# johnnyjana730/MVIN

Hardware: AMD Instinct MI355X
Metric: (user,item) pairs scored/sec @ dim=64 hop=2 fan-out=32; % HBM roofline (higher is better)
Workload: dtype f32

## Files before the change

### mvin_amd/csrc/mvin_keyaddr_flash.hip

```cpp
#include <cstdlib>
#include <type_traits>

#include "mvin_kernels.h"

namespace mvin {

typedef float f32x4 __attribute__((ext_vector_type(4)));

constexpr int kFlashChunk = 64;
constexpr int kFlashWaves = 4;

__global__ void ka_flash_slots_kernel(const int32_t* __restrict__ seg_ptr, const int32_t* __restrict__ nseg_dev, int nseg_bound,
                                      int32_t* __restrict__ slot_seg) {
    const int nseg = nseg_dev ? min(*nseg_dev, nseg_bound) : nseg_bound;
    for (int s = blockIdx.x * blockDim.x + threadIdx.x; s < nseg; s += gridDim.x * blockDim.x) {
        const int p0 = seg_ptr[s], p1 = seg_ptr[s + 1];
        const int first = p0 / kFlashChunk + s;
        const int nch = (p1 - p0 + kFlashChunk - 1) / kFlashChunk;
        for (int c = 0; c < nch; ++c) slot_seg[first + c] = s;
    }
}

#define KAF_FENCE() __builtin_amdgcn_sched_barrier(0)

__device__ long long g_kaf_trace[64 * 16];

template <int NMT, bool HAS_SET, bool TRACE = false>
__global__ __launch_bounds__(kFlashWaves * 64, 2) void key_addr_flash_kernel(KaFlashArgs a, KaRecLayout RL) {
    constexpr int D = 64;
    __shared__ f32x4 sUo0[kFlashWaves][4][64];
    const int lane = threadIdx.x & 63, l16 = lane & 15, q16 = lane >> 4;
    f32x4 (*myUo0)[64] = sUo0[threadIdx.x >> 6];
    const int P = a.P, NmP = RL.NmP;
    const unsigned emax = (unsigned)(a.n_entity - 1);
    const float* __restrict__ E = a.E;
    const size_t tw_stride = (size_t)a.n_entity * D;

    struct Rows {
        float4 v[NMT][4];
    };
    auto issue_u = [&](int mt, const int (&hr)[NMT], Rows& R) {
        const f32x4* src = reinterpret_cast<const f32x4*>(a.ER + (size_t)(unsigned)max(hr[mt], 0) * D) + q16;
#pragma unroll
        for (int nt = 0; nt < 4; ++nt) {
            const f32x4 v = __builtin_nontemporal_load(src + 4 * nt);
            R.v[mt][nt] = make_float4(v[0], v[1], v[2], v[3]);
        }
    };
    auto issue_t = [&](int mt, const float* __restrict__ tab, const int4 (&ids)[NMT], Rows& R) {
        const int id[4] = {ids[mt].x, ids[mt].y, ids[mt].z, ids[mt].w};
#pragma unroll
        for (int i = 0; i < 4; ++i)
            R.v[mt][i] = reinterpret_cast<const float4*>(tab + (size_t)(unsigned)max(id[i], 0) * D)[l16];
    };
    auto reads_tile = [&](bool two, int mt, const Rows& R, const f32x4 (&p0)[NMT], const f32x4 (&p1)[NMT], f32x4 (&u0)[4], f32x4 (&u1)[4]) {
        if (two) {
#pragma unroll
            for (int i = 0; i < 4; ++i) {
                const float t[4] = {R.v[mt][i].x, R.v[mt][i].y, R.v[mt][i].z, R.v[mt][i].w};
#pragma unroll
                for (int nt = 0; nt < 4; ++nt) u0[nt] = __builtin_amdgcn_mfma_f32_16x16x4f32(t[nt], p0[mt][i], u0[nt], 0, 0, 0);
#pragma unroll
                for (int nt = 0; nt < 4; ++nt) u1[nt] = __builtin_amdgcn_mfma_f32_16x16x4f32(t[nt], p1[mt][i], u1[nt], 0, 0, 0);
            }
        } else {
#pragma unroll
            for (int i = 0; i < 4; ++i) {
                const float t[4] = {R.v[mt][i].x, R.v[mt][i].y, R.v[mt][i].z, R.v[mt][i].w};
#pragma unroll
                for (int nt = 0; nt < 4; ++nt) u0[nt] = __builtin_amdgcn_mfma_f32_16x16x4f32(t[nt], p0[mt][i], u0[nt], 0, 0, 0);
            }
        }
    };
    auto softmax = [&](f32x4 (&lg)[NMT], const int4 (&ids)[NMT]) {
        float mx = -INFINITY;
#pragma unroll
        for (int mt = 0; mt < NMT; ++mt) {
            const int id[4] = {ids[mt].x, ids[mt].y, ids[mt].z, ids[mt].w};
#pragma unroll
            for (int i = 0; i < 4; ++i) mx = fmaxf(mx, id[i] >= 0 ? lg[mt][i] : -INFINITY);
        }
        mx = xor32_max(xor16_max(mx));
        float z = 0.f;
#pragma unroll
        for (int mt = 0; mt < NMT; ++mt) {
            const int id[4] = {ids[mt].x, ids[mt].y, ids[mt].z, ids[mt].w};
#pragma unroll
            for (int i = 0; i < 4; ++i) {
                const float x = lean_exp(fminf(lg[mt][i] - mx, 0.f));
                const float e = id[i] >= 0 ? x : 0.f;
                lg[mt][i] = e;
                z += e;
            }
        }
        z = xor32_sum(xor16_sum(z));
        const float inv = 1.f / z;
#pragma unroll
        for (int mt = 0; mt < NMT; ++mt) {
#pragma unroll
            for (int i = 0; i < 4; ++i) lg[mt][i] *= inv;
        }
    };

    int iter = 0;
    auto stamp = [&](int slot) {
        if constexpr (TRACE) {
            if (blockIdx.x == 0 && threadIdx.x == 0 && iter >= 2 && iter < 66) g_kaf_trace[(iter - 2) * 16 + slot] = __builtin_readcyclecounter();
        }
    };
    for (;; ++iter) {
        stamp(0);
        int k = 0;
        if (lane == 0) k = atomicAdd(a.counter, 1) + 1;
        k = __builtin_amdgcn_readfirstlane(k);
        if (k >= a.nslots) break;
        const int s = __builtin_amdgcn_readfirstlane(a.slot_seg[k]);
        if (s < 0) continue;
        const int u = __builtin_amdgcn_readfirstlane(a.seg_user[s]);
        const int p0 = __builtin_amdgcn_readfirstlane(a.seg_ptr[s]), p1 = __builtin_amdgcn_readfirstlane(a.seg_ptr[s + 1]);
        const int cbeg = p0 + (k - (p0 / kFlashChunk + s)) * kFlashChunk;
        const int cend = min(p1, cbeg + kFlashChunk);
        const int32_t* __restrict__ rec = a.records + (size_t)u * RL.len;
        stamp(1);
        auto load_hr = [&](int hop, int (&hr)[NMT]) {
#pragma unroll
            for (int mt = 0; mt < NMT; ++mt) hr[mt] = rec[RL.o_hr + hop * NmP + 16 * mt + l16];
        };
        auto load_tid = [&](int hop, int4 (&tid)[NMT]) {
#pragma unroll
            for (int mt = 0; mt < NMT; ++mt) tid[mt] = *reinterpret_cast<const int4*>(rec + RL.o_tail + hop * NmP + 16 * mt + 4 * q16);
        };
        auto load_orig = [&](int t0, int (&orig)[2], bool (&valid)[2]) {
#pragma unroll
            for (int rt = 0; rt < 2; ++rt) {
                const int p = t0 + 16 * rt + l16;
                valid[rt] = p < cend;
                orig[rt] = a.pair_index[min(p, cend - 1)];
            }
        };
        auto load_item = [&](const int (&orig)[2], unsigned (&item)[2]) {
#pragma unroll
            for (int rt = 0; rt < 2; ++rt)
                item[rt] = min(a.items64 ? reinterpret_cast<const unsigned*>(a.items64)[2 * (int64_t)orig[rt]] : (unsigned)a.items32[orig[rt]], emax);
        };
        auto load_be = [&](const unsigned (&item)[2], float4 (&bE)[2][4]) {
#pragma unroll
            for (int rt = 0; rt < 2; ++rt) {
#pragma unroll
                for (int nt = 0; nt < 4; ++nt) bE[rt][nt] = reinterpret_cast<const float4*>(E + (size_t)item[rt] * D)[4 * nt + q16];
            }
        };

        int orig[2], origN[2];
        bool valid[2], validN[2];
        unsigned item[2];
        float4 bE[2][4];
        int hrC[NMT], hrN[NMT];
        int4 tidC[NMT];
        Rows R;
        load_orig(cbeg, orig, valid);
        load_hr(0, hrC);
        load_tid(0, tidC);
        load_orig(cbeg + 32, origN, validN);
        f32x4 uo0[4];
#pragma unroll
        for (int r = 0; r < 4; ++r) {
            const float4 b = a.bmlp ? reinterpret_cast<const float4*>(a.bmlp)[4 * q16 + r] : make_float4(0.f, 0.f, 0.f, 0.f);
            uo0[0][r] = b.x, uo0[1][r] = b.y, uo0[2][r] = b.z, uo0[3][r] = b.w;
        }
        if constexpr (HAS_SET) {
            int4 hid[NMT];
            f32x4 ph[NMT];
#pragma unroll
            for (int mt = 0; mt < NMT; ++mt) hid[mt] = *reinterpret_cast<const int4*>(rec + RL.o_head + 16 * mt + 4 * q16);
#pragma unroll
            for (int mt = 0; mt < NMT; ++mt) issue_t(mt, a.TW, hid, R);
            KAF_FENCE();
            stamp(11);
#pragma unroll
            for (int mt = 0; mt < NMT; ++mt) {
                const int id[4] = {hid[mt].x, hid[mt].y, hid[mt].z, hid[mt].w};
#pragma unroll
                for (int i = 0; i < 4; ++i) ph[mt][i] = a.hs[max(id[i], 0)];
            }
            load_item(orig, item);
            KAF_FENCE();
            stamp(12);
            softmax(ph, hid);
            KAF_FENCE();
            stamp(13);
            f32x4 unused[4];
#pragma unroll
            for (int mt = 0; mt < NMT; ++mt) {
                reads_tile(false, mt, R, ph, ph, uo0, unused);
                KAF_FENCE();
                issue_u(mt, hrC, R);
                KAF_FENCE();
            }
            stamp(14);
        } else {
            load_item(orig, item);
#pragma unroll
            for (int mt = 0; mt < NMT; ++mt) issue_u(mt, hrC, R);
        }
        load_be(item, bE);
#pragma unroll
        for (int nt = 0; nt < 4; ++nt) myUo0[nt][lane] = uo0[nt];
        KAF_FENCE();
        stamp(2);

        const int ntile = (cend - cbeg + 31) >> 5;
        int t0 = cbeg;
        auto run_tile = [&](const bool two, const bool more) {
            f32x4 uo[2][4];
#pragma unroll
            for (int rt = 0; rt < 2; ++rt) {
#pragma unroll
                for (int nt = 0; nt < 4; ++nt) uo[rt][nt] = myUo0[nt][lane];
            }
            unsigned itemN[2];
            if (more) load_item(origN, itemN);
            for (int hop = 0; hop < P; ++hop) {
                const bool last_hop = hop + 1 == P;
                const bool next_stage = !last_hop || more;
                const int hopN = last_hop ? 0 : hop + 1;
                const float* __restrict__ tw = a.TW + (size_t)(hop + (HAS_SET ? 1 : 0)) * tw_stride;
                if (next_stage) load_hr(hopN, hrN);
                KAF_FENCE();
                if (t0 == cbeg && hop < 3) stamp(3 + 4 * hop);
                f32x4 lg[2][NMT];
#pragma unroll
                for (int mt = 0; mt < NMT; ++mt) {
                    lg[0][mt] = f32x4{0.f, 0.f, 0.f, 0.f};
                    lg[1][mt] = f32x4{0.f, 0.f, 0.f, 0.f};
                    if (two) {
#pragma unroll
                        for (int nt = 0; nt < 4; ++nt) {
                            const float av[4] = {R.v[mt][nt].x, R.v[mt][nt].y, R.v[mt][nt].z, R.v[mt][nt].w};
                            const float e0[4] = {bE[0][nt].x, bE[0][nt].y, bE[0][nt].z, bE[0][nt].w};
                            const float e1[4] = {bE[1][nt].x, bE[1][nt].y, bE[1][nt].z, bE[1][nt].w};
#pragma unroll
                            for (int i = 0; i < 4; ++i) {
                                lg[0][mt] = __builtin_amdgcn_mfma_f32_16x16x4f32(av[i], e0[i], lg[0][mt], 0, 0, 0);
                                lg[1][mt] = __builtin_amdgcn_mfma_f32_16x16x4f32(av[i], e1[i], lg[1][mt], 0, 0, 0);
                            }
                        }
                    } else {
#pragma unroll
                        for (int nt = 0; nt < 4; ++nt) {
                            const float av[4] = {R.v[mt][nt].x, R.v[mt][nt].y, R.v[mt][nt].z, R.v[mt][nt].w};
                            const float e0[4] = {bE[0][nt].x, bE[0][nt].y, bE[0][nt].z, bE[0][nt].w};
#pragma unroll
                            for (int i = 0; i < 4; ++i) lg[0][mt] = __builtin_amdgcn_mfma_f32_16x16x4f32(av[i], e0[i], lg[0][mt], 0, 0, 0);
                        }
                    }
                    KAF_FENCE();
                    issue_t(mt, tw, tidC, R);
                    KAF_FENCE();
                }
                if (last_hop && more) load_be(itemN, bE);
                KAF_FENCE();
                if (t0 == cbeg && hop < 3) stamp(4 + 4 * hop);
                softmax(lg[0], tidC);
                if (two) softmax(lg[1], tidC);
                KAF_FENCE();
                if (t0 == cbeg && hop < 3) stamp(5 + 4 * hop);
#pragma unroll
                for (int mt = 0; mt < NMT; ++mt) {
                    reads_tile(two, mt, R, lg[0], lg[1], uo[0], uo[1]);
                    KAF_FENCE();
                    if (next_stage) issue_u(mt, hrN, R);
                    KAF_FENCE();
                }
                if (next_stage) load_tid(hopN, tidC);
                if (t0 == cbeg && hop < 3) stamp(6 + 4 * hop);
            }
#pragma unroll
            for (int rt = 0; rt < 2; ++rt) {
                if (valid[rt] && (rt == 0 || two)) {
#pragma unroll
                    for (int r = 0; r < 4; ++r)
                        *reinterpret_cast<float4*>(a.user_o + (size_t)orig[rt] * D + 16 * q16 + 4 * r) =
                            make_float4(uo[rt][0][r], uo[rt][1][r], uo[rt][2][r], uo[rt][3][r]);
                }
            }
        };
        for (int tile = 0; tile < ntile; ++tile, t0 += 32) {
            const bool more = tile + 1 < ntile;
            run_tile(cend - t0 > 16, more);
#pragma unroll
            for (int rt = 0; rt < 2; ++rt) orig[rt] = origN[rt], valid[rt] = validN[rt];
        }
        stamp(15);
    }
}

hipError_t kaf_read_trace(long long* host_dst, size_t n) {
    const size_t have = sizeof(g_kaf_trace) / sizeof(long long);
    return hipMemcpyFromSymbol(host_dst, HIP_SYMBOL(g_kaf_trace), (n < have ? n : have) * sizeof(long long));
}
#undef KAF_FENCE

bool key_addr_flash_supported(int D, int P, int Nm, int nR, int n_entity) {
    if (D != 64 || P < 1 || P > 8 || Nm < 1 || Nm > 64) return false;
    const KaRecLayout RL = ka_rec_layout(P, Nm, nR);
    if (RL.len == 0) return false;
    return (long long)nR * n_entity < (1ll << 31);
}

size_t key_addr_flash_ws_elems(int64_t B, int nseg_bound) { return (size_t)(B / kFlashChunk + nseg_bound + 1) + 1; }

template <int NMT>
static hipError_t launch_flash_n(const KaFlashArgs& a, const KaRecLayout& RL, bool has_set, hipStream_t st) {
    auto k = has_set ? key_addr_flash_kernel<NMT, true> : key_addr_flash_kernel<NMT, false>;
    if constexpr (NMT == 4) {
        static const bool trace = getenv("MVIN_KAF_TRACE") != nullptr;
        if (trace && has_set) k = key_addr_flash_kernel<4, true, true>;
    }
    static thread_local int per_cu[2] = {0, 0};
    int& pc = per_cu[has_set ? 1 : 0];
    if (pc == 0) {
        int v = 0;
        if (hipOccupancyMaxActiveBlocksPerMultiprocessor(&v, reinterpret_cast<const void*>(k), kFlashWaves * 64, 0) != hipSuccess || v < 1) v = 2;
        pc = v > 8 ? 8 : v;
    }
    const int64_t want = ((int64_t)a.nslots + kFlashWaves - 1) / kFlashWaves;
    const int grid = (int)(want < 256 * (int64_t)pc ? want : 256 * (int64_t)pc);
    k<<<grid, kFlashWaves * 64, 0, st>>>(a, RL);
    return hipGetLastError();
}

hipError_t launch_key_addr_flash(const KaFlashArgs& a_, int nseg_bound, bool has_set, int32_t* sched_ws, hipStream_t st) {
    KaFlashArgs a = a_;
    const KaRecLayout RL = ka_rec_layout(a.P, a.Nm, a.nR);
    if (RL.len == 0 || !sched_ws) return hipErrorInvalidValue;
    a.nslots = (int)(a.B / kFlashChunk + nseg_bound + 1);
    a.slot_seg = sched_ws;
    a.counter = sched_ws + a.nslots;
    hipError_t e = hipMemsetAsync(sched_ws, 0xFF, ((size_t)a.nslots + 1) * sizeof(int32_t), st);
    if (e != hipSuccess) return e;
    {
        const int blocks = nseg_bound < 256 * 64 ? (nseg_bound + 255) / 256 : 64;
        ka_flash_slots_kernel<<<blocks > 0 ? blocks : 1, 256, 0, st>>>(a.seg_ptr, a.nseg_dev, nseg_bound, sched_ws);
        e = hipGetLastError();
        if (e != hipSuccess) return e;
    }
    switch (RL.NmP / 16) {
        case 1: return launch_flash_n<1>(a, RL, has_set, st);
        case 2: return launch_flash_n<2>(a, RL, has_set, st);
        case 3: return launch_flash_n<3>(a, RL, has_set, st);
        case 4: return launch_flash_n<4>(a, RL, has_set, st);
        default: return hipErrorInvalidValue;
    }
}

}
```

Measured before the change: 514.2 million.

## Prefetch next work item's records into LDS with static slot schedule

Replaces the atomic work counter with a static strided slot assignment per wave, and software-pipelines the next item's scheduling metadata, user record (head/tail/hr ids) and pair indices into double-buffered LDS via global_load_lds while the current item computes. Per-item index loads then come from LDS instead of global memory, hiding the dependent-load latency at item start. It also drops the nontemporal hint on relation-row loads and replaces the null-bias branch with a zero device buffer. The cost is LDS use that may lower occupancy, and static scheduling loses the dynamic load balancing the atomic counter gave.

Measured after the change: 534.4 million, median of 6. +3.9%, better.

```diff
diff --git a/mvin_amd/csrc/mvin_keyaddr_flash.hip b/mvin_amd/csrc/mvin_keyaddr_flash.hip
--- a/mvin_amd/csrc/mvin_keyaddr_flash.hip
+++ b/mvin_amd/csrc/mvin_keyaddr_flash.hip
@@ -23,9 +23,12 @@
 
 #define KAF_FENCE() __builtin_amdgcn_sched_barrier(0)
 
+__device__ float g_kaf_no_bias[64];
 __device__ long long g_kaf_trace[64 * 16];
 
-template <int NMT, bool HAS_SET, bool TRACE = false>
+extern __shared__ __attribute__((aligned(16))) int32_t sKafRec[];
+
+template <int NMT, bool HAS_SET, bool PF, bool TRACE = false>
 __global__ __launch_bounds__(kFlashWaves * 64, 2) void key_addr_flash_kernel(KaFlashArgs a, KaRecLayout RL) {
     constexpr int D = 64;
     __shared__ f32x4 sUo0[kFlashWaves][4][64];
@@ -34,6 +37,7 @@
     const int P = a.P, NmP = RL.NmP;
     const unsigned emax = (unsigned)(a.n_entity - 1);
     const float* __restrict__ E = a.E;
+    const float* __restrict__ bias = a.bmlp;
     const size_t tw_stride = (size_t)a.n_entity * D;
 
     struct Rows {
@@ -43,7 +47,7 @@
         const f32x4* src = reinterpret_cast<const f32x4*>(a.ER + (size_t)(unsigned)max(hr[mt], 0) * D) + q16;
 #pragma unroll
         for (int nt = 0; nt < 4; ++nt) {
-            const f32x4 v = __builtin_nontemporal_load(src + 4 * nt);
+            const f32x4 v = src[4 * nt];
             R.v[mt][nt] = make_float4(v[0], v[1], v[2], v[3]);
         }
     };
@@ -108,27 +112,147 @@
             if (blockIdx.x == 0 && threadIdx.x == 0 && iter >= 2 && iter < 66) g_kaf_trace[(iter - 2) * 16 + slot] = __builtin_readcyclecounter();
         }
     };
+    auto load_item_raw = [&](const int (&orig)[2], unsigned (&item)[2]) {
+#pragma unroll
+        for (int rt = 0; rt < 2; ++rt)
+            item[rt] = a.items64 ? reinterpret_cast<const unsigned*>(a.items64)[2 * (int64_t)orig[rt]] : (unsigned)a.items32[orig[rt]];
+    };
+    auto load_item = [&](const int (&orig)[2], unsigned (&item)[2]) {
+        load_item_raw(orig, item);
+#pragma unroll
+        for (int rt = 0; rt < 2; ++rt) item[rt] = min(item[rt], emax);
+    };
+
+    const int wave = __builtin_amdgcn_readfirstlane((int)(threadIdx.x >> 6));
+    const int stride = (int)gridDim.x * kFlashWaves;
+    const int recW = (1 + 2 * P) * NmP, ldsT = NmP, ldsHr = NmP + P * NmP;
+    const unsigned lds0 = (unsigned)(size_t)(__attribute__((address_space(3))) char*)sKafRec + (unsigned)(wave * 2 * recW * 4);
+    const int lorig = kFlashWaves * 2 * recW + wave * 32;
+    const unsigned ldsOrig = (unsigned)(size_t)(__attribute__((address_space(3))) char*)sKafRec + (unsigned)(lorig * 4);
+    auto la_slots_issue = [&](long long base) -> int {
+        const long long kc = base + (long long)stride * (lane + 1);
+        return kc < a.nslots ? a.slot_seg[kc] : -1;
+    };
+    auto la_slots_take = [&](long long base, int sv, int& kN, int& sN) -> bool {
+        for (;;) {
+            const unsigned long long live = __ballot(sv >= 0);
+            if (live) {
+                const int j = __ffsll(live) - 1;
+                kN = __builtin_amdgcn_readfirstlane((int)(base + (long long)stride * (j + 1)));
+                sN = __builtin_amdgcn_readlane(sv, j);
+                return true;
+            }
+            base += 64ll * stride;
+            if (base + stride >= a.nslots) return false;
+            sv = la_slots_issue(base);
+        }
+    };
+    auto la_seg_issue = [&](int s) -> int {
+        const int32_t* src = lane == 0 ? a.seg_user + s : a.seg_ptr + s + (lane - 1);
+        return lane < 3 ? *src : 0;
+    };
+    auto la_seg_take = [&](int v, int k, int s, int& u, int& cbeg, int& cend) {
+        u = __builtin_amdgcn_readlane(v, 0);
+        const int p0 = __builtin_amdgcn_readlane(v, 1), p1 = __builtin_amdgcn_readlane(v, 2);
+        cbeg = p0 + (k - (p0 / kFlashChunk + s)) * kFlashChunk;
+        cend = min(p1, cbeg + kFlashChunk);
+    };
+    auto la_rec_issue = [&](int u, int cbeg, int cend, int par) {
+        const char* src = reinterpret_cast<const char*>(a.records + (size_t)u * RL.len);
+        const unsigned dst = lds0 + (unsigned)(par * recW * 4);
+        for (int j0 = 0; j0 < recW; j0 += 64) {
+            const int i = j0 + lane;
+            if (i < recW) {
+                const int voff = 4 * (i < NmP ? RL.o_head + i : RL.o_tail + (i - NmP));
+                unsigned keep;
+                asm volatile("s_nop 4\n\ts_mov_b32 %0, m0\n\ts_mov_b32 m0, %3\n\ts_nop 0\n\tglobal_load_lds_dword %1, %2\n\ts_mov_b32 m0, %0"
+                             : "=&s"(keep)
+                             : "v"(voff), "s"(src), "s"(dst + 4u * (unsigned)j0)
+                             : "memory");
+            }
+        }
+        if (lane < 32) {
+            const int voff = 4 * min(lane, cend - 1 - cbeg);
+            unsigned keep;
+            asm volatile("s_nop 4\n\ts_mov_b32 %0, m0\n\ts_mov_b32 m0, %3\n\ts_nop 0\n\tglobal_load_lds_dword %1, %2\n\ts_mov_b32 m0, %0"
+                         : "=&s"(keep)
+                         : "v"(voff), "s"(a.pair_index + cbeg), "s"(ldsOrig)
+                         : "memory");
+        }
+    };
+    auto la_orig = [&](int (&orig)[2]) {
+#pragma unroll
+        for (int rt = 0; rt < 2; ++rt) orig[rt] = sKafRec[lorig + 16 * rt + l16];
+    };
+    bool nHave = false;
+    int nK = 0, nS = 0, nU = 0, nCbeg = 0, nCend = 0;
+    int par = 0;
+    int laSlots = 0, laSeg = 0;
+    unsigned itemP[2] = {0, 0};
+    if constexpr (PF) {
+        const long long base = (long long)((int)blockIdx.x * kFlashWaves + wave) - stride;
+        nHave = la_slots_take(base, la_slots_issue(base), nK, nS);
+        if (nHave) {
+            la_seg_take(la_seg_issue(nS), nK, nS, nU, nCbeg, nCend);
+            la_rec_issue(nU, nCbeg, nCend, par);
+            asm volatile("s_waitcnt vmcnt(0)" ::: "memory");
+            int o[2];
+            la_orig(o);
+            load_item_raw(o, itemP);
+        }
+    }
     for (;; ++iter) {
         stamp(0);
-        int k = 0;
-        if (lane == 0) k = atomicAdd(a.counter, 1) + 1;
-        k = __builtin_amdgcn_readfirstlane(k);
-        if (k >= a.nslots) break;
-        const int s = __builtin_amdgcn_readfirstlane(a.slot_seg[k]);
-        if (s < 0) continue;
-        const int u = __builtin_amdgcn_readfirstlane(a.seg_user[s]);
-        const int p0 = __builtin_amdgcn_readfirstlane(a.seg_ptr[s]), p1 = __builtin_amdgcn_readfirstlane(a.seg_ptr[s + 1]);
-        const int cbeg = p0 + (k - (p0 / kFlashChunk + s)) * kFlashChunk;
-        const int cend = min(p1, cbeg + kFlashChunk);
+        int k = 0, u = 0, cbeg = 0, cend = 0;
+        if constexpr (PF) {
+            if (!nHave) break;
+            k = nK, u = nU, cbeg = nCbeg, cend = nCend;
+            asm volatile("s_waitcnt vmcnt(0)" ::: "memory");
+        } else {
+            if (lane == 0) k = atomicAdd(a.counter, 1) + 1;
+            k = __builtin_amdgcn_readfirstlane(k);
+            if (k >= a.nslots) break;
+            const int s = __builtin_amdgcn_readfirstlane(a.slot_seg[k]);
+            if (s < 0) continue;
+            u = __builtin_amdgcn_readfirstlane(a.seg_user[s]);
+            const int p0 = __builtin_amdgcn_readfirstlane(a.seg_ptr[s]), p1 = __builtin_amdgcn_readfirstlane(a.seg_ptr[s + 1]);
+            cbeg = p0 + (k - (p0 / kFlashChunk + s)) * kFlashChunk;
+            cend = min(p1, cbeg + kFlashChunk);
+        }
         const int32_t* __restrict__ rec = a.records + (size_t)u * RL.len;
+        const int lrec = (wave * 2 + par) * recW;
         stamp(1);
         auto load_hr = [&](int hop, int (&hr)[NMT]) {
 #pragma unroll
-            for (int mt = 0; mt < NMT; ++mt) hr[mt] = rec[RL.o_hr + hop * NmP + 16 * mt + l16];
+            for (int mt = 0; mt < NMT; ++mt) {
+                if constexpr (PF) hr[mt] = sKafRec[lrec + ldsHr + hop * NmP + 16 * mt + l16];
+                else hr[mt] = rec[RL.o_hr + hop * NmP + 16 * mt + l16];
+            }
         };
         auto load_tid = [&](int hop, int4 (&tid)[NMT]) {
 #pragma unroll
-            for (int mt = 0; mt < NMT; ++mt) tid[mt] = *reinterpret_cast<const int4*>(rec + RL.o_tail + hop * NmP + 16 * mt + 4 * q16);
+            for (int mt = 0; mt < NMT; ++mt) {
+                if constexpr (PF) tid[mt] = *reinterpret_cast<const int4*>(&sKafRec[lrec + ldsT + hop * NmP + 16 * mt + 4 * q16]);
+                else tid[mt] = *reinterpret_cast<const int4*>(rec + RL.o_tail + hop * NmP + 16 * mt + 4 * q16);
+            }
+        };
+        auto la_step_slots = [&]() {
+            nHave = la_slots_take(k, laSlots, nK, nS);
+            if (nHave) laSeg = la_seg_issue(nS);
+        };
+        auto la_step_seg = [&]() {
+            if (nHave) {
+                la_seg_take(laSeg, nK, nS, nU, nCbeg, nCend);
+                la_rec_issue(nU, nCbeg, nCend, par ^ 1);
+            }
+        };
+        auto la_step_items = [&](bool rows_since) {
+            if (nHave) {
+                if (!rows_since) asm volatile("s_waitcnt vmcnt(0)" ::: "memory");
+                int o[2];
+                la_orig(o);
+                load_item_raw(o, itemP);
+            }
         };
         auto load_orig = [&](int t0, int (&orig)[2], bool (&valid)[2]) {
 #pragma unroll
@@ -137,11 +261,6 @@
                 valid[rt] = p < cend;
                 orig[rt] = a.pair_index[min(p, cend - 1)];
             }
-        };
-        auto load_item = [&](const int (&orig)[2], unsigned (&item)[2]) {
-#pragma unroll
-            for (int rt = 0; rt < 2; ++rt)
-                item[rt] = min(a.items64 ? reinterpret_cast<const unsigned*>(a.items64)[2 * (int64_t)orig[rt]] : (unsigned)a.items32[orig[rt]], emax);
         };
         auto load_be = [&](const unsigned (&item)[2], float4 (&bE)[2][4]) {
 #pragma unroll
@@ -158,34 +277,48 @@
         int hrC[NMT], hrN[NMT];
         int4 tidC[NMT];
         Rows R;
-        load_orig(cbeg, orig, valid);
+        if constexpr (PF) {
+#pragma unroll
+            for (int rt = 0; rt < 2; ++rt) item[rt] = min(itemP[rt], emax), valid[rt] = cbeg + 16 * rt + l16 < cend;
+            la_orig(orig);
+        } else {
+            load_orig(cbeg, orig, valid);
+        }
         load_hr(0, hrC);
         load_tid(0, tidC);
         load_orig(cbeg + 32, origN, validN);
         f32x4 uo0[4];
 #pragma unroll
         for (int r = 0; r < 4; ++r) {
-            const float4 b = a.bmlp ? reinterpret_cast<const float4*>(a.bmlp)[4 * q16 + r] : make_float4(0.f, 0.f, 0.f, 0.f);
+            const float4 b = reinterpret_cast<const float4*>(bias)[4 * q16 + r];
             uo0[0][r] = b.x, uo0[1][r] = b.y, uo0[2][r] = b.z, uo0[3][r] = b.w;
         }
         if constexpr (HAS_SET) {
             int4 hid[NMT];
             f32x4 ph[NMT];
 #pragma unroll
-            for (int mt = 0; mt < NMT; ++mt) hid[mt] = *reinterpret_cast<const int4*>(rec + RL.o_head + 16 * mt + 4 * q16);
+            for (int mt = 0; mt < NMT; ++mt) {
+                if constexpr (PF) hid[mt] = *reinterpret_cast<const int4*>(&sKafRec[lrec + 16 * mt + 4 * q16]);
+                else hid[mt] = *reinterpret_cast<const int4*>(rec + RL.o_head + 16 * mt + 4 * q16);
+            }
 #pragma unroll
             for (int mt = 0; mt < NMT; ++mt) issue_t(mt, a.TW, hid, R);
             KAF_FENCE();
             stamp(11);
+            if constexpr (PF) laSlots = la_slots_issue(k);
 #pragma unroll
             for (int mt = 0; mt < NMT; ++mt) {
                 const int id[4] = {hid[mt].x, hid[mt].y, hid[mt].z, hid[mt].w};
 #pragma unroll
                 for (int i = 0; i < 4; ++i) ph[mt][i] = a.hs[max(id[i], 0)];
             }
-            load_item(orig, item);
+            if constexpr (!PF) load_item(orig, item);
             KAF_FENCE();
             stamp(12);
+            if constexpr (PF) {
+                la_step_slots();
+                KAF_FENCE();
+            }
             softmax(ph, hid);
             KAF_FENCE();
             stamp(13);
@@ -199,11 +332,16 @@
             }
             stamp(14);
         } else {
-            load_item(orig, item);
+            if constexpr (!PF) load_item(orig, item);
 #pragma unroll
             for (int mt = 0; mt < NMT; ++mt) issue_u(mt, hrC, R);
+            if constexpr (PF) laSlots = la_slots_issue(k);
         }
         load_be(item, bE);
+        if constexpr (PF && !HAS_SET) {
+            KAF_FENCE();
+            la_step_slots();
+        }
 #pragma unroll
         for (int nt = 0; nt < 4; ++nt) myUo0[nt][lane] = uo0[nt];
         KAF_FENCE();
@@ -211,6 +349,16 @@
 
         const int ntile = (cend - cbeg + 31) >> 5;
         int t0 = cbeg;
+        int stage = 0;
+        const int stage_items = min(2, 2 * ntile * P - 1);
+        auto la_stage = [&]() {
+            if constexpr (PF) {
+                if (stage == 0) la_step_seg();
+                if (stage == stage_items) la_step_items(stage_items == 2);
+                ++stage;
+                KAF_FENCE();
+            }
+        };
         auto run_tile = [&](const bool two, const bool more) {
             f32x4 uo[2][4];
 #pragma unroll
@@ -261,6 +409,7 @@
                 if (last_hop && more) load_be(itemN, bE);
                 KAF_FENCE();
                 if (t0 == cbeg && hop < 3) stamp(4 + 4 * hop);
+                la_stage();
                 softmax(lg[0], tidC);
                 if (two) softmax(lg[1], tidC);
                 KAF_FENCE();
@@ -274,6 +423,7 @@
                 }
                 if (next_stage) load_tid(hopN, tidC);
                 if (t0 == cbeg && hop < 3) stamp(6 + 4 * hop);
+                la_stage();
             }
 #pragma unroll
             for (int rt = 0; rt < 2; ++rt) {
@@ -292,6 +442,7 @@
             for (int rt = 0; rt < 2; ++rt) orig[rt] = origN[rt], valid[rt] = validN[rt];
         }
         stamp(15);
+        par ^= 1;
     }
 }
 
@@ -310,23 +461,33 @@
 
 size_t key_addr_flash_ws_elems(int64_t B, int nseg_bound) { return (size_t)(B / kFlashChunk + nseg_bound + 1) + 1; }
 
+static int env_int(const char* name, int dflt) {
+    const char* v = getenv(name);
+    return v && *v ? atoi(v) : dflt;
+}
+
 template <int NMT>
 static hipError_t launch_flash_n(const KaFlashArgs& a, const KaRecLayout& RL, bool has_set, hipStream_t st) {
-    auto k = has_set ? key_addr_flash_kernel<NMT, true> : key_addr_flash_kernel<NMT, false>;
+    static const bool prefetch = env_int("MVIN_KAF_PREFETCH", 1) != 0;
+    static const int grid_cap = env_int("MVIN_KAF_GRID", 0);
+    auto k = prefetch ? (has_set ? key_addr_flash_kernel<NMT, true, true> : key_addr_flash_kernel<NMT, false, true>)
+                      : (has_set ? key_addr_flash_kernel<NMT, true, false> : key_addr_flash_kernel<NMT, false, false>);
     if constexpr (NMT == 4) {
         static const bool trace = getenv("MVIN_KAF_TRACE") != nullptr;
-        if (trace && has_set) k = key_addr_flash_kernel<4, true, true>;
-    }
-    static thread_local int per_cu[2] = {0, 0};
-    int& pc = per_cu[has_set ? 1 : 0];
+        if (trace && has_set) k = prefetch ? key_addr_flash_kernel<4, true, true, true> : key_addr_flash_kernel<4, true, false, true>;
+    }
+    const size_t lds = prefetch ? (size_t)kFlashWaves * (2 * (1 + 2 * a.P) * RL.NmP + 32) * sizeof(int32_t) : 0;
+    static thread_local int per_cu[2][9] = {};
+    int& pc = per_cu[has_set ? 1 : 0][a.P];
     if (pc == 0) {
         int v = 0;
-        if (hipOccupancyMaxActiveBlocksPerMultiprocessor(&v, reinterpret_cast<const void*>(k), kFlashWaves * 64, 0) != hipSuccess || v < 1) v = 2;
+        if (hipOccupancyMaxActiveBlocksPerMultiprocessor(&v, reinterpret_cast<const void*>(k), kFlashWaves * 64, lds) != hipSuccess || v < 1) v = 2;
         pc = v > 8 ? 8 : v;
     }
     const int64_t want = ((int64_t)a.nslots + kFlashWaves - 1) / kFlashWaves;
-    const int grid = (int)(want < 256 * (int64_t)pc ? want : 256 * (int64_t)pc);
-    k<<<grid, kFlashWaves * 64, 0, st>>>(a, RL);
+    int grid = (int)(want < 256 * (int64_t)pc ? want : 256 * (int64_t)pc);
+    if (grid_cap > 0 && grid > grid_cap) grid = grid_cap;
+    k<<<grid, kFlashWaves * 64, lds, st>>>(a, RL);
     return hipGetLastError();
 }
 
@@ -334,6 +495,11 @@
     KaFlashArgs a = a_;
     const KaRecLayout RL = ka_rec_layout(a.P, a.Nm, a.nR);
     if (RL.len == 0 || !sched_ws) return hipErrorInvalidValue;
+    if (!a.bmlp) {
+        void* zeros = nullptr;
+        if (hipError_t e = hipGetSymbolAddress(&zeros, HIP_SYMBOL(g_kaf_no_bias)); e != hipSuccess) return e;
+        a.bmlp = static_cast<const float*>(zeros);
+    }
     a.nslots = (int)(a.B / kFlashChunk + nseg_bound + 1);
     a.slot_seg = sched_ws;
     a.counter = sched_ws + a.nslots;
```
